# COMP6248-Reproducability-Challenge/selfsupervised-denoising

Measured on AMD Instinct MI355X. Metric: training patches/sec (64x64 gauss25 SSDN), higher is better.
Workload: dtype f16

## Files before the change

### selfsupervised-denoising_amd/csrc/common.h

```cpp
#pragma once
#include <hip/hip_runtime.h>
#include <hip/hip_ext.h>
#include <stdint.h>
#include "../../include/ssdn_hip.h"
#include <cstdlib>

#if defined(SSDN_TUNING)
static inline const char* ssdn_tuning_env(const char* name) { return std::getenv(name); }
#else
static inline const char* ssdn_tuning_env(const char*) { return nullptr; }
#endif

typedef _Float16 h16;
typedef _Float16 half8 __attribute__((ext_vector_type(8)));
typedef _Float16 half4 __attribute__((ext_vector_type(4)));
typedef _Float16 half2v __attribute__((ext_vector_type(2)));
typedef __bf16 bf16x8 __attribute__((ext_vector_type(8)));
typedef unsigned short u16x8 __attribute__((ext_vector_type(8)));
typedef unsigned short u16x4 __attribute__((ext_vector_type(4)));
typedef float f32x16 __attribute__((ext_vector_type(16)));
typedef float f32x4 __attribute__((ext_vector_type(4)));

#define LRELU_SLOPE 0.1f

// ... 111 lines not shown
int launch_adam(const ssdn_adam_args* a, hipStream_t s);
#define ADAM_PACK_MAX 24
int adam_pack_fusable(const ssdn_adam_args* a, const ssdn_wpack_args* const* items, int n);
int launch_adam_pack(const ssdn_adam_args* a, const ssdn_wpack_args* const* items, int n, hipStream_t s);
int launch_metrics(const ssdn_metrics_args* a, hipStream_t s);
int launch_accum(const ssdn_accum_args* a, hipStream_t s);
int launch_noise(const ssdn_noise_args* a, hipStream_t s);
int launch_input_grad(const ssdn_input_grad_args* a, hipStream_t s);
int conv_lds_bytes(const ssdn_conv_args* a);
int conv_validate(const ssdn_conv_args* a);
int chain_len(const ssdn_op* ops, int n, bool any_lane);
int launch_chain(const ssdn_op* ops, int n, bool any_lane, hipStream_t s);
bool chain_merging_on();
bool conv_dma_eligible(const ssdn_conv_args* a, bool any_size);
int conv_dma_lds_bytes(int mt);
bool conv_signs(const ssdn_conv_args* a);
bool gemm_dma_signs(const ssdn_conv_args* a);
bool conv_dma_signs(const ssdn_conv_args* a);
bool conv_fuses_urot(const ssdn_conv_args* a);
bool conv_fuses_unrot(const ssdn_conv_args* a);
bool conv_fuses_upsum(const ssdn_conv_args* a);
bool conv_fuses_pool(const ssdn_conv_args* a);
int launch_conv_dma(const ssdn_conv_args* a, hipStream_t s);
bool conv_thin_eligible(const ssdn_conv_args* a);
bool conv_thin_fuses_pack(const ssdn_pack_input_args* pk, const ssdn_conv_args* a);
int launch_conv_thin(const ssdn_conv_args* a, const ssdn_pack_input_args* pk, hipStream_t s);
bool conv_pack_fusable(const ssdn_pack_input_args* pk, const ssdn_conv_args* a);
bool gradpack_dgrad_fusable(const ssdn_grad_pack_args* gp, const ssdn_conv_args* a);
int launch_gradpack_dgrad(const ssdn_grad_pack_args* gp, const ssdn_conv_args* a, hipStream_t s);
bool conv_gradpack_fusable(const ssdn_grad_pack_args* gp, const ssdn_conv_args* a);
bool gemm_dma_eligible(const ssdn_conv_args* a);
int gemm_dma_lds_bytes(const ssdn_conv_args* a);
int launch_gemm_dma(const ssdn_conv_args* a, hipStream_t s);
bool gemm_dma_fuses_next(const ssdn_conv_args* a, const ssdn_conv_args* b);
int launch_gemm_dma_with_next(const ssdn_conv_args* a, const ssdn_conv_args* b, hipStream_t s);
bool conv_pair_fusable(const ssdn_conv_args* a, const ssdn_conv_args* b);
extern "C" int ssdn_device_cus(void);
int wgrad_lds_bytes(const ssdn_wgrad_args* a);
```

### selfsupervised-denoising_amd/csrc/conv_dma.hip

```cpp
#include "common.h"
#include <cstdlib>
#include <type_traits>
#include <utility>

#if defined(SSDN_CDMA_TUNING) || defined(SSDN_TUNING)
#define CD_ABL(xx, bit) (((xx).ablate & (bit)) != 0)
#define CD_TUNING 1
#else
#define CD_ABL(xx, bit) false
#define CD_TUNING 0
#endif

#ifndef CD_DEPHASE
#define CD_DEPHASE 0
#endif
#ifndef CD_MOVE_BARRIER
#define CD_MOVE_BARRIER 1
#endif
#ifndef CD_WARMUP
#define CD_WARMUP 1
#endif

namespace {

constexpr int CD_TBYTES = 31744;

struct CdAux {
    int m_base, m_cnt;
    int padT, padL, rev;
    int tiles_x, tiles_y;
    int segs, tps;
    int segs_sh;
    unsigned tx_magic;
    int nitems, xcd_map;
    int nfull, tail16;
    int ablate;
    int wrep;
    int dephase;
    unsigned long long* trace;
};

typedef __attribute__((address_space(3))) void* cd_lds_ptr;
__device__ __forceinline__ void dma16(unsigned lds_addr, int voff, __amdgpu_buffer_rsrc_t rs, int soff) {
    __builtin_amdgcn_raw_ptr_buffer_load_lds(rs, (cd_lds_ptr)(size_t)__builtin_amdgcn_readfirstlane(lds_addr), 16, voff, __builtin_amdgcn_readfirstlane(soff), 0, 0);
}

template <bool BF>
__device__ __forceinline__ void cd_mma(f32x16& c, half8 av, half8 bv) {
    if constexpr (BF) c = __builtin_amdgcn_mfma_f32_32x32x16_bf16(__builtin_bit_cast(bf16x8, av), __builtin_bit_cast(bf16x8, bv), c, 0, 0, 0);
    else c = __builtin_amdgcn_mfma_f32_32x32x16_f16(av, bv, c, 0, 0, 0);
}
// ... 46 lines not shown
template <int IMM, int AUX = 0>
__device__ __forceinline__ void dma16i(unsigned lds_addr, int voff, __amdgpu_buffer_rsrc_t rs, int soff) {
    __builtin_amdgcn_raw_ptr_buffer_load_lds(rs, (cd_lds_ptr)(size_t)lds_addr, 16, voff, soff, IMM, AUX);
}

}

template <int MT, bool BF, int EPI, int KIND>
__global__ __launch_bounds__(256, 2) void k_cdma(ssdn_conv_args a, CdAux x) {
    constexpr bool AF = KIND == 1;
    extern __shared__ __attribute__((aligned(16))) char smem[];
    constexpr int WROWS = MT * 32;
    constexpr int WBYTES = WROWS * 96;
    constexpr int OSTR = MT * 64 + 16;
    constexpr int NEK = MT * 2;
    constexpr bool HAS_MASK = (EPI & 1) != 0, HAS_ADD = (EPI & 2) != 0, HAS_UPS = (EPI & 4) != 0, UROT = (EPI & 8) != 0;
    constexpr bool SOUT = (EPI & 16) != 0, SMASK = (EPI & 32) != 0;
    constexpr int NUK = (8 * MT * 4 + 63) / 64;
    constexpr int G = 2 * MT;
    constexpr bool MOVE = CD_MOVE_BARRIER != 0;
    const int tid = threadIdx.x, lane = tid & 63, l31 = lane & 31, kh = lane >> 5;
    const int w = __builtin_amdgcn_readfirstlane(tid >> 6);
    const bool wload = w < 2;
    const int lw = w & 1;
    const unsigned lds0 = (unsigned)(size_t)smem;
    char* const tbuf0 = smem;
    const unsigned tlds0 = lds0, wlds0 = lds0 + 2 * CD_TBYTES;

    const int G_ = gridDim.x;
    int it_first, it_stride, it_end;
    if (x.xcd_map) {
        const int i8 = x.nitems >> 3, xcd = blockIdx.x & 7;
        it_first = xcd * i8 + (blockIdx.x >> 3); it_stride = G_ >> 3; it_end = (xcd + 1) * i8;
    } else {
        it_first = blockIdx.x; it_stride = G_; it_end = x.nitems;
    }
    if (it_first >= it_end) return;
#if CD_WARMUP
    const int pf_line = (blockIdx.x >> 3) * 256 + tid;
    const unsigned pf = __builtin_amdgcn_raw_buffer_load_b32(
        __builtin_amdgcn_make_buffer_rsrc(const_cast<void*>(a.wc), 0, 9 * a.Mpad * a.Ktot * 2, SSDN_BUFFER_RSRC_FLAGS), pf_line << 7, 0, 0);
#endif

    const int bE48 = (4 * w + (l31 >> 4)) * 1728 + (l31 & 15) * 96 + ((kh ^ ((l31 >> 4) & 1)) << 4);
    const int aB48 = l31 * 96 + ((kh ^ ((l31 >> 3) & 1)) << 4);
    const int cpp = x.m_cnt >> 3;

    const __amdgpu_buffer_rsrc_t rs_wc = __builtin_amdgcn_make_buffer_rsrc(const_cast<void*>(a.wc), 0, (int)0x80000000, SSDN_BUFFER_RSRC_FLAGS);
    const int H0 = a.up0 ? (a.H >> 1) : a.H, W0 = a.up0 ? (a.W >> 1) : a.W;
    const int nch = x.nfull + x.tail16;

    int tr_i = 0;
    auto stamp = [&]() __attribute__((always_inline)) {
        if (CD_TUNING && x.trace && tid == 0 && tr_i < 32) x.trace[(size_t)blockIdx.x * 32 + tr_i++] = __builtin_amdgcn_s_memtime();
    };

    const int wtap = a.Mpad * a.Ktot * 2;
    const int wt0 = x.rev ? 8 * wtap : 0, wts = x.rev ? -wtap : wtap;
    const int wvoff = lane * 16;
    const bool lw0 = __builtin_amdgcn_readfirstlane(tid >> 6) == 0;
    auto wchunk = [&](int c) __attribute__((always_inline)) {
        return __builtin_amdgcn_readfirstlane((c * 48 * a.Mpad + x.m_base * ((AF || c < x.nfull) ? 48 : 16)) * 2 + wt0);
    };
    auto wpiece = [&](auto FULLc, auto Jc, unsigned d, int so) __attribute__((always_inline)) {
        using S = CdWSplit<MT, decltype(FULLc)::value != 0>;
        constexpr int j = decltype(Jc)::value;
        if (CD_ABL(x, 2)) return;
        if constexpr (j < S::NB) dma16i<j * 1024>(d, wvoff, rs_wc, so);
        else if constexpr (S::extra) { if (lw0) dma16i<0>(d + 2 * S::NB * 1024, wvoff, rs_wc, so + 2 * S::NB * 1024); }
    };
    auto wbase = [&](bool full) __attribute__((always_inline)) {
        return lw ? (full ? CdWSplit<MT, true>::b1 : CdWSplit<MT, false>::b1) * 1024 : 0;
    };
    auto wslice = [&](bool full, unsigned dbuf, int sl) __attribute__((always_inline)) {
        const int wb = wbase(full);
        if (AF || full) cd_static_for<CdWSplit<MT, true>::NB + 1>([&](auto jc) { wpiece(cd_ic<1>{}, jc, dbuf + wb, sl + wb); });
        else cd_static_for<CdWSplit<MT, false>::NB + 1>([&](auto jc) { wpiece(cd_ic<0>{}, jc, dbuf + wb, sl + wb); });
    };

    __amdgpu_buffer_rsrc_t rs_t = rs_wc;
    int t_so = 0, t_incA = 0, t_incB = 0, t_ybs = 0, rlE = 0, rlO = 0;
    unsigned t_tb = 0;
    auto tile_setup = [&](int tn, int ty0, int tx0, int c, int tbi, bool live) __attribute__((always_inline)) {
        const int k0 = c * 48;
        const bool from0 = k0 < a.c0;
// ... 32 lines not shown
            int voff = (hy & 1) ? rlO : rlE;
            if constexpr (hy < 2 || hy >= 16) voff = (unsigned)(t_ybs + hy) < (unsigned)a.H ? voff : (int)0x80000000;
            if (CD_ABL(x, 512)) dma16i<0, 2>(t_tb + hy * 1728, voff, rs_t, so);
            else dma16i<0>(t_tb + hy * 1728, voff, rs_t, so);
        } else {
            int voff = lw ? rlO : rlE;
            voff = (unsigned)(t_ybs + lw + 2 * hy) < (unsigned)a.H ? voff : (int)0x80000000;
            if (lane < 36) dma16i<0>(t_tb + hy * 1152, voff, rs_t, so);
        }
    };

    auto tile_of = [&](int item, int k) {
        const int strip = item >> x.segs_sh, seg = item & (x.segs - 1);
        CdTile t;
        t.n = x.tiles_x == 1 ? strip : (int)__umulhi((unsigned)strip, x.tx_magic);
        t.x0 = (strip - t.n * x.tiles_x) * 16;
        t.y0 = (seg * x.tps + k) * 16;
        return t;
    };
    int item = it_first, kt = 0;
    CdTile cur = tile_of(item, 0);
    int tpar = 0, wpar = 0;
    float* const bl = reinterpret_cast<float*>(smem + 18 * 18 * 96);
    if (tid < WROWS) bl[tid] = (a.bias && tid < x.m_cnt) ? a.bias[x.m_base + tid] : 0.f;
    constexpr int CD_LUT = 18 * 18 * 96 + 384;
    static_assert(CD_LUT + 256 <= CD_TBYTES && WROWS * 4 <= 384, "pad behind tile buffer 0");
    if constexpr (SMASK && HAS_MASK) {
        if (tid < 64) reinterpret_cast<float*>(smem + CD_LUT)[tid] = ((tid >> 2) >> (tid & 3)) & 1 ? 1.f : LRELU_SLOPE;
    }

    const __amdgpu_buffer_rsrc_t rs_dst = __builtin_amdgcn_make_buffer_rsrc(UROT ? a.urot.p : a.dst.p, 0, CD_ABL(x, 64) ? 0 : (int)0x80000000, SSDN_BUFFER_RSRC_FLAGS);
    const __amdgpu_buffer_rsrc_t rs_sgn = __builtin_amdgcn_make_buffer_rsrc(SOUT ? a.sign_out : a.urot_smask, 0, (!CD_ABL(x, 64) && (SOUT || (UROT && a.urot_smask))) ? (int)0x80000000 : 0, SSDN_BUFFER_RSRC_FLAGS);
    const __amdgpu_buffer_rsrc_t rs_ms = __builtin_amdgcn_make_buffer_rsrc(const_cast<void*>(HAS_UPS ? a.upsum_mask_sign : a.mask_sign), 0, SMASK ? (int)0x80000000 : 0, SSDN_BUFFER_RSRC_FLAGS);
    const float slope = a.act ? LRELU_SLOPE : 1.f;
    const __amdgpu_buffer_rsrc_t rs_mask = __builtin_amdgcn_make_buffer_rsrc(a.mask.p, 0, HAS_MASK ? (int)0x80000000 : 0, SSDN_BUFFER_RSRC_FLAGS);
    const __amdgpu_buffer_rsrc_t rs_add = __builtin_amdgcn_make_buffer_rsrc(a.add.p, 0, HAS_ADD ? (int)0x80000000 : 0, SSDN_BUFFER_RSRC_FLAGS);
    const __amdgpu_buffer_rsrc_t rs_up = __builtin_amdgcn_make_buffer_rsrc(a.upsum.p, 0, HAS_UPS ? (int)0x80000000 : 0, SSDN_BUFFER_RSRC_FLAGS);
    const __amdgpu_buffer_rsrc_t rs_um = __builtin_amdgcn_make_buffer_rsrc(a.upsum_mask.p, 0, HAS_UPS ? (int)0x80000000 : 0, SSDN_BUFFER_RSRC_FLAGS);
    int u_pc[NUK];
#pragma unroll
    for (int k = 0; k < NUK; ++k) {
        const int p = k * 64 + lane;
        const int j = p / cpp, c = p - j * cpp;
        u_pc[k] = p < 8 * cpp ? (j | (c << 8)) : -1;
    }

    auto run = [&](auto WLc) __attribute__((always_inline)) {
// ... 164 lines not shown
        if (!CD_ABL(x, 8) && !HAS_UPS && (cpp & 1) == 0 && !CD_ABL(x, 1024)) {
            const int pix_t = (cur.n * a.H + cur.y0 + 4 * w) * a.W + cur.x0;
            const int npair = __builtin_amdgcn_readfirstlane(cpp >> 1);
            int lane_o = lane;
            asm volatile("" : "+v"(lane_o));
            const int l31 = lane_o & 31, kh = lane_o >> 5;
            const int lrow = l31 >> 4, lcol = l31 & 15;
            const int lpix = lrow * a.W + lcol;
            int ur_base = 0, ur_iu = 0, ur_iv = 0, ur_ju = 0, ur_jv = 0;
            if constexpr (UROT) {
                const int Bq = a.N >> 2, P1 = a.H - 1;
                const int r = (cur.n >= Bq ? 1 : 0) + (cur.n >= 2 * Bq ? 1 : 0) + (cur.n >= 3 * Bq ? 1 : 0);
                ur_iu = r == 0 ? 1 : (r == 2 ? -1 : 0); ur_iv = r == 1 ? 1 : (r == 3 ? -1 : 0);
                ur_ju = r == 3 ? 1 : (r == 1 ? -1 : 0); ur_jv = r == 0 ? 1 : (r == 2 ? -1 : 0);
                const int i0 = r >= 2 ? P1 : 0, j0 = (r == 1 || r == 2) ? P1 : 0;
                ur_base = (((cur.n - r * Bq) * a.H + i0) * a.W + j0) * a.urot.cs + a.urot.co + r * a.M;
            }
            constexpr bool HOIST = HAS_MASK && SMASK && !HAS_ADD && !UROT;
            unsigned mbh[2][MT * 2];
            if constexpr (HOIST) {
#pragma unroll
                for (int nt = 0; nt < 2; ++nt) {
                    const int pix_p = pix_t + 2 * nt * a.W;
                    const int s_so = __builtin_amdgcn_readfirstlane(pix_p * (a.M >> 3) + (x.m_base >> 3));
#pragma unroll
                    for (int i = 0; i < MT * 2; ++i) {
                        if (i >= npair) break;
                        mbh[nt][i] = __builtin_amdgcn_raw_buffer_load_b8(rs_ms, lpix * (a.M >> 3) + kh + i * 2, s_so, 0);
                    }
                }
            }
            auto pass = [&](auto NtC, auto ActC) __attribute__((always_inline)) {
                constexpr int nt = decltype(NtC)::value;
                constexpr bool ACTC = decltype(ActC)::value != 0;
                const int pix_p = pix_t + 2 * nt * a.W;
                int d_lane, d_so = 0;
                bool live = true;
                if constexpr (UROT) {
                    const int u = cur.y0 + 4 * w + 2 * nt + lrow + 1, v = cur.x0 + lcol;
                    live = u < a.H;
                    const int dpx = (ur_iu * u + ur_iv * v) * a.W + ur_ju * u + ur_jv * v;
                    d_lane = live ? (ur_base + dpx * a.urot.cs + x.m_base) * 2 + kh * 16 : (int)0x80000000;
                } else {
                    d_lane = lpix * a.dst.cs * 2 + kh * 16;
                    d_so = __builtin_amdgcn_readfirstlane((pix_p * a.dst.cs + a.dst.co + x.m_base) * 2);
                }
                const int s_lane = live ? lpix * (a.M >> 3) + kh : (int)0x80000000;
                const int s_so = __builtin_amdgcn_readfirstlane(pix_p * (a.M >> 3) + (x.m_base >> 3));
                u32x4_t ab[MT * 2], mb[MT * 2];
#pragma unroll
                for (int i = 0; i < MT * 2; ++i) {
                    if (i >= npair) break;
                    if constexpr (HAS_ADD)
                        ab[i] = __builtin_amdgcn_raw_buffer_load_b128(rs_add, lpix * a.add.cs * 2 + kh * 16 + i * 32,
                                                                      __builtin_amdgcn_readfirstlane((pix_p * a.add.cs + a.add.co + x.m_base) * 2), 0);
                    if constexpr (HOIST)
                        mb[i][0] = mbh[nt][i];
                    else if constexpr (HAS_MASK && SMASK)
                        mb[i][0] = __builtin_amdgcn_raw_buffer_load_b8(rs_ms, s_lane + i * 2, s_so, 0);
                    else if constexpr (HAS_MASK)
                        mb[i] = __builtin_amdgcn_raw_buffer_load_b128(rs_mask, lpix * a.mask.cs * 2 + kh * 16 + i * 32,
                                                                      __builtin_amdgcn_readfirstlane((pix_p * a.mask.cs + a.mask.co + x.m_base) * 2), 0);
                }
#pragma unroll
                for (int mt = 0; mt < MT; ++mt)
#pragma unroll
                    for (int gp = 0; gp < 2; ++gp) {
                        constexpr int DUMMY = 0; (void)DUMMY;
                        const int i = mt * 2 + gp;
                        if (i >= npair) break;
                        unsigned pk[2][2];
#pragma unroll
                        for (int h = 0; h < 2; ++h) {
                            float v[4];
#pragma unroll
                            for (int j = 0; j < 4; ++j) v[j] = acc[mt][nt][(2 * gp + h) * 4 + j];
                            if constexpr (ACTC) {
#pragma unroll
                                for (int j = 0; j < 4; j += 2) {
                                    const f32x2_t t = f32x2_t{v[j], v[j + 1]} * LRELU_SLOPE;
                                    asm("v_max_f32 %0, %1, %2" : "=v"(v[j]) : "v"(v[j]), "v"(t[0]));
                                    asm("v_max_f32 %0, %1, %2" : "=v"(v[j + 1]) : "v"(v[j + 1]), "v"(t[1]));
                                }
                            }
                            pk[h][0] = BF ? pack_bf16x2(v[0], v[1]) : pack_f16x2(v[0], v[1]);
// ... 83 lines not shown
                const int Bq = a.N >> 2, P1 = a.H - 1;
                const int r = (cur.n >= Bq ? 1 : 0) + (cur.n >= 2 * Bq ? 1 : 0) + (cur.n >= 3 * Bq ? 1 : 0);
                ur_iu = r == 0 ? 1 : (r == 2 ? -1 : 0); ur_iv = r == 1 ? 1 : (r == 3 ? -1 : 0);
                ur_ju = r == 3 ? 1 : (r == 1 ? -1 : 0); ur_jv = r == 0 ? 1 : (r == 2 ? -1 : 0);
                const int i0 = r >= 2 ? P1 : 0, j0 = (r == 1 || r == 2) ? P1 : 0;
                ur_base = (((cur.n - r * Bq) * a.H + i0) * a.W + j0) * a.urot.cs + a.urot.co + r * a.M;
            }
#pragma unroll
            for (int nt = 0; nt < 2; ++nt) {
                const int pix_p = pix_t + 2 * nt * a.W;
                u32x4_t ab[NEK], mb[NEK];
                int goff[NEK], soff[NEK];
#pragma unroll
                for (int k = 0; k < NEK; ++k) {
                    int epc = e_pc[k];
                    asm volatile("" : "+v"(epc));
                    const bool on = epc >= 0;
                    const int px = epc & 255, c16 = (epc >> 8) << 4;
                    const int pix = pix_p + (px >> 4) * a.W + (px & 15);
                    if constexpr (UROT) {
                        const int u = cur.y0 + 4 * w + 2 * nt + (px >> 4) + 1, v = cur.x0 + (px & 15);
                        const bool live = on && u < a.H;
                        const int dpx = (ur_iu * u + ur_iv * v) * a.W + ur_ju * u + ur_jv * v;
                        goff[k] = live ? (ur_base + dpx * a.urot.cs + x.m_base) * 2 + c16 : (int)0x80000000;
                        soff[k] = live ? pix * (a.M >> 3) + (x.m_base >> 3) + (c16 >> 4) : (int)0x80000000;
                    } else
                    goff[k] = on ? (pix * a.dst.cs + a.dst.co + x.m_base) * 2 + c16 : (int)0x80000000;
                    if constexpr (HAS_ADD)
                        ab[k] = __builtin_amdgcn_raw_buffer_load_b128(rs_add, on ? (pix * a.add.cs + a.add.co + x.m_base) * 2 + c16 : (int)0x80000000, 0, 0);
                    if constexpr (HAS_MASK && SMASK)
                        mb[k][0] = __builtin_amdgcn_raw_buffer_load_b8(rs_ms, on ? pix * (a.M >> 3) + (x.m_base >> 3) + (c16 >> 4) : (int)0x80000000, 0, 0);
                    else if constexpr (HAS_MASK)
                        mb[k] = __builtin_amdgcn_raw_buffer_load_b128(rs_mask, on ? (pix * a.mask.cs + a.mask.co + x.m_base) * 2 + c16 : (int)0x80000000, 0, 0);
                    if constexpr (SOUT) soff[k] = on ? pix * (a.M >> 3) + (x.m_base >> 3) + (c16 >> 4) : (int)0x80000000;
                }
#pragma unroll
                for (int mt = 0; mt < MT; ++mt)
#pragma unroll
                    for (int gp = 0; gp < 2; ++gp) {
                        unsigned pk[2][2];
#pragma unroll
                        for (int h = 0; h < 2; ++h) {
                            float v[4];
#pragma unroll
                            for (int j = 0; j < 4; ++j) v[j] = acc[mt][nt][(2 * gp + h) * 4 + j];
                            if constexpr (!BF) {
#pragma unroll
                                for (int j = 0; j < 4; j += 2) {
                                    const f32x2_t t = f32x2_t{v[j], v[j + 1]} * slope;
                                    asm("v_max_f32 %0, %1, %2" : "=v"(v[j]) : "v"(v[j]), "v"(t[0]));
                                    asm("v_max_f32 %0, %1, %2" : "=v"(v[j + 1]) : "v"(v[j + 1]), "v"(t[1]));
                                }
                            }
                            pk[h][0] = BF ? pack_bf16x2(v[0], v[1]) : pack_f16x2(v[0], v[1]);
                            pk[h][1] = BF ? pack_bf16x2(v[2], v[3]) : pack_f16x2(v[2], v[3]);
                        }
                        u32x4_t o;
#pragma unroll
                        for (int d = 0; d < 2; ++d) {
                            auto r = __builtin_amdgcn_permlane32_swap(pk[0][d], pk[1][d], false, false);
                            o[d] = r[0]; o[2 + d] = r[1];
                        }
                        const int piece = mt * 4 + 2 * gp + kh;
                        *reinterpret_cast<u32x4_t*>(reg + l31 * OSTR + piece * 16) = o;
                    }
                if constexpr (HAS_UPS) {
                    const int pixl = (cur.n * (a.H >> 1) + ((cur.y0 + 4 * w + 2 * nt) >> 1)) * (a.W >> 1) + (cur.x0 >> 1);
                    u32x4_t um[NUK];
#pragma unroll
                    for (int k = 0; k < NUK; ++k) {
                        int upc = u_pc[k];
                        asm volatile("" : "+v"(upc));
                        const bool on = upc >= 0;
                        const int j = upc & 255, c16 = (upc >> 8) << 4;
                        if constexpr (SMASK)
                            um[k][0] = __builtin_amdgcn_raw_buffer_load_b8(rs_ms, on ? (pixl + j) * (a.upsum_c >> 3) + (x.m_base >> 3) + (c16 >> 4) : (int)0x80000000, 0, 0);
                        else
                        um[k] = __builtin_amdgcn_raw_buffer_load_b128(rs_um, on ? ((pixl + j) * a.upsum_mask.cs + a.upsum_mask.co + x.m_base) * 2 + c16 : (int)0x80000000, 0, 0);
                    }
#pragma unroll
                    for (int k = 0; k < NUK; ++k) {
                        int upc = u_pc[k];
                        asm volatile("" : "+v"(upc));
                        const bool on = upc >= 0;
                        const int j = upc & 255, c16 = (upc >> 8) << 4;
                        float sum[8] = {0.f, 0.f, 0.f, 0.f, 0.f, 0.f, 0.f, 0.f};
#pragma unroll
                        for (int q4 = 0; q4 < 4; ++q4) {
                            const u32x4_t o = *reinterpret_cast<const u32x4_t*>(reg + (on ? ((q4 >> 1) * 16 + 2 * j + (q4 & 1)) * OSTR + c16 : 0));
#pragma unroll
                            for (int q = 0; q < 4; ++q) { sum[2 * q] += bf_lo(o[q]); sum[2 * q + 1] += bf_hi(o[q]); }
                        }
                        u32x4_t r;
#pragma unroll
                        for (int q = 0; q < 4; ++q) {
                            int mlo, mhi;
                            if constexpr (SMASK) { mlo = (um[k][0] >> (2 * q)) & 1u; mhi = (um[k][0] >> (2 * q + 1)) & 1u; }
                            else { mlo = (int)(short)(um[k][q] & 0xffffu); mhi = (int)um[k][q] >> 16; }
                            r[q] = pack_bf16x2(sum[2 * q] * (mlo > 0 ? 1.f : LRELU_SLOPE), sum[2 * q + 1] * (mhi > 0 ? 1.f : LRELU_SLOPE));
                        }
                        __builtin_amdgcn_raw_buffer_store_b128(r, rs_up, on ? ((pixl + j) * a.upsum.cs + a.upsum.co + x.m_base) * 2 + c16 : (int)0x80000000, 0, 0);
                    }
                } else {
#pragma unroll
                for (int k = 0; k < NEK; ++k) {
                    int epc = e_pc[k];
                    asm volatile("" : "+v"(epc));
                    const bool on = epc >= 0;
                    const int px = epc & 255, c16 = (epc >> 8) << 4;
                    u32x4_t o = *reinterpret_cast<const u32x4_t*>(reg + (on ? px * OSTR + c16 : 0));
                    if constexpr (HAS_MASK || HAS_ADD) {
#pragma unroll
                        for (int q = 0; q < 4; ++q) {
                            float v0, v1;
                            if constexpr (BF) {
                                v0 = bf_lo(o[q]); v1 = bf_hi(o[q]);
                                if constexpr (HAS_ADD) { v0 += bf_lo(ab[k][q]); v1 += bf_hi(ab[k][q]); }
                            } else {
                                v0 = f16_lo(o[q]); v1 = f16_hi(o[q]);
                                if constexpr (HAS_ADD) { v0 += f16_lo(ab[k][q]); v1 += f16_hi(ab[k][q]); }
                            }
                            if constexpr (HAS_MASK) {
                                int mlo, mhi;
                                if constexpr (SMASK) { mlo = (mb[k][0] >> (2 * q)) & 1u; mhi = (mb[k][0] >> (2 * q + 1)) & 1u; }
// ... 42 lines not shown
        if (i != 2 - t / 3 || j != 2 - t % 3) mir = false;
    }
    if (!fwd && !mir) return false;
    *padT = -mny; *padL = -mnx; *rev = fwd ? 0 : 1;
    return true;
}

bool conv_dma_eligible(const ssdn_conv_args* a, bool any_size) {
    int pt, pl, rv;
    if (!cd_window(a, &pt, &pl, &rv)) return false;
    if (a->dst32 || (a->H & 15) || (a->W & 15) || !a->wc) return false;
    const int tail = a->Ktot % 48;
    if (tail != 0 && tail != 16) return false;
    if (a->c0 % 48 && a->c0 != a->Ktot) return false;
    if ((a->M & 7) || (a->Mpad & 31)) return false;
    if (!a->bf16 && (a->mask.p || a->add.p)) return false;
    if (a->bf16 && a->act) return false;
    if (a->urot.p && (a->bf16 || a->M != 96 || a->Mpad != 96 || a->H != a->W || (a->N & 3) || a->mask.p || a->add.p || a->upsum.p || a->pool.p ||
                      (a->urot.co & 7) || (a->urot.cs & 7) || (long long)(a->N / 4) * a->H * a->W * a->urot.cs * 2 >= (1ll << 31))) return false;
    if (a->upsum.p && (!a->bf16 || a->mask.p || a->add.p || a->upsum_c % 96 || a->upsum_c > a->M)) return false;
    int cus = ssdn_device_cus();
    if (cus <= 0) cus = 256;
    const long long tiles = (long long)a->N * (a->H >> 4) * (a->W >> 4);
    if (!(tiles >= cus || (2 * tiles >= cus && a->H * a->W > 256)) && !any_size) return false;
    if ((long long)a->N * (a->W >> 4) >= 65536) return false;
    int csmax = a->dst.cs > a->src1.cs ? a->dst.cs : a->src1.cs;
    csmax = csmax > a->src0.cs ? csmax : a->src0.cs;
    csmax = csmax > a->mask.cs ? csmax : a->mask.cs;
    csmax = csmax > a->add.cs ? csmax : a->add.cs;
    if ((long long)a->N * a->H * a->W * csmax * 2 >= (1ll << 31)) return false;
    if (9ll * a->Mpad * a->Ktot * 2 >= (1ll << 31)) return false;
    return true;
}

bool conv_dma_signs(const ssdn_conv_args* a) {
    if (!conv_dma_eligible(a, false)) return false;
    if (a->sign_out && (a->bf16 || !a->dst.p || a->urot.p || a->M != 96 || a->Mpad != 96)) return false;
    if (a->mask_sign && (!a->bf16 || !a->mask.p || a->add.p || a->upsum.p || a->mask.cs != a->M || a->mask.co != 0 || (a->Mpad != 96 && a->Mpad != 64))) return false;
    if (a->upsum_mask_sign && (!a->bf16 || !a->upsum.p || a->upsum_mask.cs != a->upsum_c || a->upsum_mask.co != 0)) return false;
    return true;
}

int conv_dma_lds_bytes(int mt) { return 2 * CD_TBYTES + 2 * mt * 32 * 96; }

template <int MT, bool BF, int EPI, int KIND>
static int cd_launch_kind(const ssdn_conv_args* a, CdAux x, hipStream_t s) {
    static bool attr_set_dev[SSDN_MAX_DEVICES_ATTR] = {};
    bool& attr_set = attr_set_dev[ssdn_current_device_slot()];
    if (!attr_set) {
        SSDN_CHECK_HIP(hipFuncSetAttribute((const void*)k_cdma<MT, BF, EPI, KIND>, hipFuncAttributeMaxDynamicSharedMemorySize, 160 * 1024));
        attr_set = true;
    }
    int cus = ssdn_device_cus();
    if (cus <= 0) return -1;
    const int nstrips = a->N * x.tiles_x;
    x.segs = 1;
    while (nstrips * x.segs < 2 * cus && x.segs < x.tiles_y && x.tiles_y % (x.segs * 2) == 0) x.segs *= 2;
    x.tps = x.tiles_y / x.segs;
    x.segs_sh = 0;
    while ((1 << x.segs_sh) < x.segs) ++x.segs_sh;
    x.tx_magic = x.tiles_x > 1 ? (unsigned)((0x100000000ull + x.tiles_x - 1) / x.tiles_x) : 0u;
    x.nitems = nstrips * x.segs;
    const int grid = x.nitems < 2 * cus ? x.nitems : 2 * cus;
    x.xcd_map = (x.nitems % 8 == 0 && grid % 8 == 0) ? 1 : 0;
    const double px = (double)a->N * a->H * a->W;
    const int kreal = a->kreal > 0 ? a->kreal : a->Ktot;
    const double flops = 2.0 * px * x.m_cnt * kreal * 9;
    const double bytes = px * (a->c0 * 2.0 / (a->up0 ? 4.0 : 1.0) + a->c1 * 2.0) + px * x.m_cnt * 2.0;
    prof_begin(MT == 3 ? SSDN_PROF_CDMA_MT3 : SSDN_PROF_CDMA_MT21, s);
    SSDN_LAUNCH((k_cdma<MT, BF, EPI, KIND>), dim3(grid), dim3(256), conv_dma_lds_bytes(MT), s, *a, x);
    prof_end(MT == 3 ? SSDN_PROF_CDMA_MT3 : SSDN_PROF_CDMA_MT21, s, flops, bytes);
    return 0;
}
template <int MT, bool BF, int EPI>
static int cd_launch(const ssdn_conv_args* a, const CdAux& x, hipStream_t s) {
    if (x.tail16 == 0 && x.nfull > 0) return cd_launch_kind<MT, BF, EPI, 1>(a, x, s);
    if constexpr (!BF) {
        if (x.tail16 == 1 && x.nfull > 0) return cd_launch_kind<MT, BF, EPI, 2>(a, x, s);
    }
    return cd_launch_kind<MT, BF, EPI, 0>(a, x, s);
}

template <int MT>
static int cd_launch_role(const ssdn_conv_args* a, const CdAux& x, hipStream_t s) {
    if (a->urot.p) {
        if constexpr (MT == 3) return cd_launch<3, false, 8>(a, x, s);
        return ssdn_set_error("conv_dma: fused UNROT_FWD needs M = 96");
    }
    if (!a->bf16) {
        if (a->sign_out) {
            if constexpr (MT == 3) return cd_launch<3, false, 16>(a, x, s);
            return ssdn_set_error("conv_dma: sign_out needs M = 96");
        }
// ... 3 lines not shown
        if constexpr (MT == 3) {
            if (x.m_base + 96 <= a->upsum_c && x.m_cnt == 96 && !a->mask.p && !a->add.p)
                return a->upsum_mask_sign ? cd_launch<3, true, 4 | 32>(a, x, s) : cd_launch<3, true, 4>(a, x, s);
        }
        return ssdn_set_error("conv_dma: fused upsum needs whole 96-channel blocks without mask / add");
    }
    const int epi = (a->mask.p ? 1 : 0) | (a->add.p ? 2 : 0);
    if (a->mask_sign) {
        if constexpr (MT >= 2) { if (epi == 1) return cd_launch<MT, true, 1 | 32>(a, x, s); }
        return ssdn_set_error("conv_dma: mask_sign needs a mask, no skip gradient, Mpad = 96 or 64");
    }
    switch (epi) {
        case 0: return cd_launch<MT, true, 0>(a, x, s);
        case 1: return cd_launch<MT, true, 1>(a, x, s);
        case 2: return cd_launch<MT, true, 2>(a, x, s);
        default: return cd_launch<MT, true, 3>(a, x, s);
    }
}

int launch_conv_dma(const ssdn_conv_args* a, hipStream_t s) {
    CdAux x;
    if (!cd_window(a, &x.padT, &x.padL, &x.rev)) return ssdn_set_error("conv_dma: not a 3x3 window");
    x.tiles_x = a->W >> 4; x.tiles_y = a->H >> 4;
    x.segs = 1; x.tps = x.tiles_y; x.nitems = 0; x.xcd_map = 0; x.segs_sh = 0; x.tx_magic = 0;
    x.nfull = a->Ktot / 48; x.tail16 = (a->Ktot % 48) ? 1 : 0;
    static const int env_ablate = [] { const char* e = ssdn_tuning_env("SSDN_CDMA_ABLATE"); return e ? atoi(e) : 0; }();
    x.ablate = env_ablate;
    static const int env_wrep = [] { const char* e = ssdn_tuning_env("SSDN_CDMA_WREP"); return e ? atoi(e) : 0; }();
    x.wrep = env_wrep;
    static const int env_dephase = [] { const char* e = ssdn_tuning_env("SSDN_CDMA_DEPHASE"); return e ? atoi(e) : CD_DEPHASE; }();
    x.dephase = env_dephase;
    x.trace = (unsigned long long*)ssdn_debug_get_trace();
    int rc = 0;
    for (int mb = 0; mb < a->Mpad && !rc; mb += 96) {
        int rows = a->Mpad - mb;
        rows = rows > 96 ? 96 : rows;
        const int mt = rows / 32;
        x.m_base = mb;
        x.m_cnt = a->M - mb < rows ? a->M - mb : rows;
        if (x.m_cnt <= 0) break;
        if (mt == 3) rc = cd_launch_role<3>(a, x, s);
        else if (mt == 2) rc = cd_launch_role<2>(a, x, s);
        else rc = cd_launch_role<1>(a, x, s);
    }
    if (rc) return rc;
    SSDN_CHECK_HIP(hipGetLastError());
    return 0;
}

#endif
```

### selfsupervised-denoising_amd/csrc/conv_mfma.hip

```cpp
#include "common.h"
#ifdef SSDN_TUNING
#define CV_ABL(xx, bit) (((xx).ablate & (bit)) != 0)
#define CV_TUNING 1
#else
#define CV_ABL(xx, bit) false
#define CV_TUNING 0
#endif
#include <cstdlib>


struct ConvGeom {
    int TW, TH, TN, HH, HW, padT, padB, padL, padR;
    int PSTR, WSTR, NP;
    int tiles_x, tiles_y, groups_n;
};

static __host__ __device__ inline ConvGeom conv_geom(int ltw, int lth, int ltn, int ntaps, const int* dy, const int* dx,
                                                     int N, int H, int W, int kc) {
    ConvGeom g;
    g.TW = 1 << ltw; g.TH = 1 << lth; g.TN = 1 << ltn;
    int mny = 0, mxy = 0, mnx = 0, mxx = 0;
    for (int t = 0; t < ntaps; ++t) {
        mny = dy[t] < mny ? dy[t] : mny; mxy = dy[t] > mxy ? dy[t] : mxy;
        mnx = dx[t] < mnx ? dx[t] : mnx; mxx = dx[t] > mxx ? dx[t] : mxx;
// ... 634 lines not shown
                        v1 *= lrelu_grad(f16_hi(mb[w]));
                    }
                    o[w] = BF ? pack_bf16x2(v0, v1) : pack_f16x2(v0, v1);
                }
            }
            __builtin_amdgcn_raw_buffer_store_b128(o, rd[u], go[u], 0, 0);
        }
    }
    stamp();
}

static bool conv_uses_mt1(const ssdn_conv_args* a, const ConvGeom& g) {
    static int mt1_tiles = -1;
    if (mt1_tiles < 0) {
        const char* e = ssdn_tuning_env("SSDN_CONV_MT1_TILES");
        mt1_tiles = e ? atoi(e) : ssdn_device_cus();
        if (mt1_tiles <= 0) mt1_tiles = 256;
    }
    return !a->dst32 && g.tiles_x * g.tiles_y * g.groups_n <= mt1_tiles && a->Mpad >= 64;
}

static int g_conv_mode = [] { const char* e = ssdn_tuning_env("SSDN_CONV_DMA"); return e ? atoi(e) : 1; }();
extern "C" int ssdn_conv_set_mode(int mode) {
    if (mode < 0 || mode > 2) return ssdn_set_error("conv mode must be 0, 1 or 2");
    g_conv_mode = mode;
    return 0;
}
static bool conv_use_dma(const ssdn_conv_args* a) { return g_conv_mode > 0 && !a->pool.p && conv_dma_eligible(a, g_conv_mode == 2); }
static bool conv_use_gemm(const ssdn_conv_args* a) { return g_conv_mode > 0 && gemm_dma_eligible(a); }
static bool conv_use_thin(const ssdn_conv_args* a) { return g_conv_mode > 0 && conv_thin_eligible(a); }
bool conv_gradpack_fusable(const ssdn_grad_pack_args* gp, const ssdn_conv_args* a) {
    return !conv_validate(a) && !conv_use_gemm(a) && !conv_use_thin(a) && !conv_use_dma(a) && gradpack_dgrad_fusable(gp, a);
}
bool conv_pair_fusable(const ssdn_conv_args* a, const ssdn_conv_args* b) {
    return !conv_validate(a) && !conv_validate(b) && conv_use_gemm(a) && gemm_dma_fuses_next(a, b);
}
bool conv_pack_fusable(const ssdn_pack_input_args* pk, const ssdn_conv_args* a) {
    return !conv_validate(a) && !conv_use_gemm(a) && conv_use_thin(a) && conv_thin_fuses_pack(pk, a);
}

int conv_validate(const ssdn_conv_args* a) {
    if (a->ntaps < 1 || a->ntaps > SSDN_MAX_TAPS) return ssdn_set_error("conv: ntaps out of range");
    if (a->ltw + a->lth + a->ltn > 9 || a->ltw < 0 || a->lth < 0 || a->ltn < 0) return ssdn_set_error("conv: tile must have <= 512 pixels");
    if (a->Ktot != a->c0 + a->c1 || (a->Ktot & 15)) return ssdn_set_error("conv: Ktot must equal c0+c1 and be a multiple of 16");
    if ((a->c0 & 7) || (a->c1 & 7)) return ssdn_set_error("conv: source channel counts must be multiples of 8");
    if (a->kc < 16 || (a->kc & 15) || a->Ktot % a->kc || (a->kc > 64 && a->kc != 96)) return ssdn_set_error("conv: kc must be 16, 32, 48, 64 or 96 and divide Ktot");
    if ((a->Mpad & 31) || a->M > a->Mpad) return ssdn_set_error("conv: Mpad must be a multiple of 32 and >= M");
    if (!a->dst32 && ((a->M & 7) || (a->dst.co & 7) || (a->dst.cs & 7))) return ssdn_set_error("conv: 16-bit output needs M, dst.co, dst.cs %% 8 == 0");
    if (a->add.p && ((a->add.co & 7) || (a->add.cs & 7))) return ssdn_set_error("conv: add view must be 16-byte aligned");
    if (a->mask.p && ((a->mask.co & 7) || (a->mask.cs & 7))) return ssdn_set_error("conv: mask view must be 16-byte aligned");
// ... 164 lines not shown
```

### selfsupervised-denoising_amd/ssdn/hip/graph.py

```python
from __future__ import annotations

import os
from dataclasses import dataclass, field
from typing import Dict, List, Optional, Set, Tuple

LDS_LIMIT = 160 * 1024
CONV_LDS_PREFERRED = 80 * 1024
WGRAD_SMALL_PX = 32768
SMALL_WGRAD_G, SMALL_WGRAD_CUS = 2, 64
MID_WGRAD_PX, MID_WGRAD_G = 131072, 2
WGRAD_CU_FRAC = (3, 4)
WGRAD_MEGA = "split"
FUSE_UNROT_FWD = True
SIGN_BYTES_HEAD = True
X16_SLOTS = 16
POOL_ROUTE = True
SIGN_BYTES_CONV = True
SIGN_BYTES = True
MEGA_MIN_PX = 32768
SPLIT_HEAD_CUS = (1, 2)
SPLIT_AFTER = "decode_block_2.2"
SPLIT_GROUP0 = ("output_block", "decode_block_2.2")
MEGA_LANE = 0
WGRAD_LANE = 1
# ... 146 lines not shown


def _behind_runs(at: Dict[int, int], runs, only=None) -> None:
    for first, end in runs:
        for k in at:
            if first <= at[k] < end and (only is None or k in only):
                at[k] = end



def _pads(taps):
    dys = [t[0] for t in taps]
    dxs = [t[1] for t in taps]
    return max(0, -min(dys)), max(0, max(dys)), max(0, -min(dxs)), max(0, max(dxs))


def _pow2ceil_log(v: int) -> int:
    l = 0
    while (1 << l) < v:
        l += 1
    return l


def cdma_fills(tiles: int, cus: int, H: int = 0, W: int = 0) -> bool:
    return tiles >= cus or (2 * tiles >= cus and H * W > 256)


def choose_conv_tile(N, H, W, taps, Ktot, Mpad, budget=LDS_LIMIT, out16=True, cus=256):
    padT, padB, padL, padR = _pads(taps)
    best = None
    for ltw in range(0, min(5, _pow2ceil_log(W)) + 1):
        for lth in range(0, min(8 - ltw, _pow2ceil_log(H)) + 1):
            for ltn in range(0, min(8 - ltw - lth, _pow2ceil_log(N)) + 1):
                TW, TH, TN = 1 << ltw, 1 << lth, 1 << ltn
                tiles = -(-W // TW) * -(-H // TH) * -(-N // TN)
                util = (N * H * W) / (tiles * 256.0)
                NP = TN * (TH + padT + padB) * (TW + padL + padR)
                mt1 = out16 and tiles <= cus and Mpad >= 64
                mt = 1 if mt1 else min(3, Mpad // 32)
                kcs = [kc for kc in ((16, 32, 48, 64, 96) if mt1 else (16, 32, 48, 64)) if Ktot % kc == 0]
                for kc in kcs:
                    lds = NP * (kc * 2 + 16) + 2 * mt * 32 * (kc * 2 + 16)
                    if len(taps) == 1 and Ktot // kc >= 2:
                        lds = max(lds, 2 * NP * kc * 2 + 2 * mt * 32 * (kc * 2 + 16))
                    if out16:
                        lds = max(lds, TN * TH * TW * (mt * 64 + 16) + mt * 128)
                    if lds > budget:
                        continue
# ... 594 lines not shown
```

Measured before the change: 20570.

## Split M=96 forward DMA conv across grid.y to fill CUs on small grids

Adds an output-channel split for plain M=96 forward convs in the DMA conv kernel: when too few spatial strips exist to fill twice the CU count, it launches an MT=1 kernel with three blocks in grid.y, each handling 32 output rows. It also relaxes DMA-conv eligibility for f16 (non-bf16) convs to require only 2*tiles >= CUs, so more small layers take this path. The aim is better CU occupancy on low-resolution layers, at the cost of rereading input tiles three times and using a narrower MMA tile per block. A Python helper mirrors the relaxed eligibility, and a new conv mode 3 disables the split.

```diff
diff --git a/selfsupervised-denoising_amd/csrc/common.h b/selfsupervised-denoising_amd/csrc/common.h
--- a/selfsupervised-denoising_amd/csrc/common.h
+++ b/selfsupervised-denoising_amd/csrc/common.h
@@ -157,6 +157,7 @@
 bool conv_fuses_upsum(const ssdn_conv_args* a);
 bool conv_fuses_pool(const ssdn_conv_args* a);
 int launch_conv_dma(const ssdn_conv_args* a, hipStream_t s);
+int conv_mode_now();
 bool conv_thin_eligible(const ssdn_conv_args* a);
 bool conv_thin_fuses_pack(const ssdn_pack_input_args* pk, const ssdn_conv_args* a);
 int launch_conv_thin(const ssdn_conv_args* a, const ssdn_pack_input_args* pk, hipStream_t s);
diff --git a/selfsupervised-denoising_amd/csrc/conv_dma.hip b/selfsupervised-denoising_amd/csrc/conv_dma.hip
--- a/selfsupervised-denoising_amd/csrc/conv_dma.hip
+++ b/selfsupervised-denoising_amd/csrc/conv_dma.hip
@@ -27,6 +27,7 @@
 
 struct CdAux {
     int m_base, m_cnt;
+    int msplit;
     int padT, padL, rev;
     int tiles_x, tiles_y;
     int segs, tps;
@@ -119,6 +120,7 @@
     const int tid = threadIdx.x, lane = tid & 63, l31 = lane & 31, kh = lane >> 5;
     const int w = __builtin_amdgcn_readfirstlane(tid >> 6);
     const bool wload = w < 2;
+    const int m_base = MT == 1 ? x.m_base + (int)blockIdx.y * 32 : x.m_base;
     const int lw = w & 1;
     const unsigned lds0 = (unsigned)(size_t)smem;
     char* const tbuf0 = smem;
@@ -157,7 +159,7 @@
     const int wvoff = lane * 16;
     const bool lw0 = __builtin_amdgcn_readfirstlane(tid >> 6) == 0;
     auto wchunk = [&](int c) __attribute__((always_inline)) {
-        return __builtin_amdgcn_readfirstlane((c * 48 * a.Mpad + x.m_base * ((AF || c < x.nfull) ? 48 : 16)) * 2 + wt0);
+        return __builtin_amdgcn_readfirstlane((c * 48 * a.Mpad + m_base * ((AF || c < x.nfull) ? 48 : 16)) * 2 + wt0);
     };
     auto wpiece = [&](auto FULLc, auto Jc, unsigned d, int so) __attribute__((always_inline)) {
         using S = CdWSplit<MT, decltype(FULLc)::value != 0>;
@@ -236,7 +238,7 @@
     CdTile cur = tile_of(item, 0);
     int tpar = 0, wpar = 0;
     float* const bl = reinterpret_cast<float*>(smem + 18 * 18 * 96);
-    if (tid < WROWS) bl[tid] = (a.bias && tid < x.m_cnt) ? a.bias[x.m_base + tid] : 0.f;
+    if (tid < WROWS) bl[tid] = (a.bias && tid < x.m_cnt) ? a.bias[m_base + tid] : 0.f;
     constexpr int CD_LUT = 18 * 18 * 96 + 384;
     static_assert(CD_LUT + 256 <= CD_TBYTES && WROWS * 4 <= 384, "pad behind tile buffer 0");
     if constexpr (SMASK && HAS_MASK) {
@@ -447,7 +449,7 @@
 #pragma unroll
                 for (int nt = 0; nt < 2; ++nt) {
                     const int pix_p = pix_t + 2 * nt * a.W;
-                    const int s_so = __builtin_amdgcn_readfirstlane(pix_p * (a.M >> 3) + (x.m_base >> 3));
+                    const int s_so = __builtin_amdgcn_readfirstlane(pix_p * (a.M >> 3) + (m_base >> 3));
 #pragma unroll
                     for (int i = 0; i < MT * 2; ++i) {
                         if (i >= npair) break;
@@ -465,27 +467,27 @@
                     const int u = cur.y0 + 4 * w + 2 * nt + lrow + 1, v = cur.x0 + lcol;
                     live = u < a.H;
                     const int dpx = (ur_iu * u + ur_iv * v) * a.W + ur_ju * u + ur_jv * v;
-                    d_lane = live ? (ur_base + dpx * a.urot.cs + x.m_base) * 2 + kh * 16 : (int)0x80000000;
+                    d_lane = live ? (ur_base + dpx * a.urot.cs + m_base) * 2 + kh * 16 : (int)0x80000000;
                 } else {
                     d_lane = lpix * a.dst.cs * 2 + kh * 16;
-                    d_so = __builtin_amdgcn_readfirstlane((pix_p * a.dst.cs + a.dst.co + x.m_base) * 2);
+                    d_so = __builtin_amdgcn_readfirstlane((pix_p * a.dst.cs + a.dst.co + m_base) * 2);
                 }
                 const int s_lane = live ? lpix * (a.M >> 3) + kh : (int)0x80000000;
-                const int s_so = __builtin_amdgcn_readfirstlane(pix_p * (a.M >> 3) + (x.m_base >> 3));
+                const int s_so = __builtin_amdgcn_readfirstlane(pix_p * (a.M >> 3) + (m_base >> 3));
                 u32x4_t ab[MT * 2], mb[MT * 2];
 #pragma unroll
                 for (int i = 0; i < MT * 2; ++i) {
                     if (i >= npair) break;
                     if constexpr (HAS_ADD)
                         ab[i] = __builtin_amdgcn_raw_buffer_load_b128(rs_add, lpix * a.add.cs * 2 + kh * 16 + i * 32,
-                                                                      __builtin_amdgcn_readfirstlane((pix_p * a.add.cs + a.add.co + x.m_base) * 2), 0);
+                                                                      __builtin_amdgcn_readfirstlane((pix_p * a.add.cs + a.add.co + m_base) * 2), 0);
                     if constexpr (HOIST)
                         mb[i][0] = mbh[nt][i];
                     else if constexpr (HAS_MASK && SMASK)
                         mb[i][0] = __builtin_amdgcn_raw_buffer_load_b8(rs_ms, s_lane + i * 2, s_so, 0);
                     else if constexpr (HAS_MASK)
                         mb[i] = __builtin_amdgcn_raw_buffer_load_b128(rs_mask, lpix * a.mask.cs * 2 + kh * 16 + i * 32,
-                                                                      __builtin_amdgcn_readfirstlane((pix_p * a.mask.cs + a.mask.co + x.m_base) * 2), 0);
+                                                                      __builtin_amdgcn_readfirstlane((pix_p * a.mask.cs + a.mask.co + m_base) * 2), 0);
                 }
 #pragma unroll
                 for (int mt = 0; mt < MT; ++mt)
@@ -615,17 +617,17 @@
                         const int u = cur.y0 + 4 * w + 2 * nt + (px >> 4) + 1, v = cur.x0 + (px & 15);
                         const bool live = on && u < a.H;
                         const int dpx = (ur_iu * u + ur_iv * v) * a.W + ur_ju * u + ur_jv * v;
-                        goff[k] = live ? (ur_base + dpx * a.urot.cs + x.m_base) * 2 + c16 : (int)0x80000000;
-                        soff[k] = live ? pix * (a.M >> 3) + (x.m_base >> 3) + (c16 >> 4) : (int)0x80000000;
+                        goff[k] = live ? (ur_base + dpx * a.urot.cs + m_base) * 2 + c16 : (int)0x80000000;
+                        soff[k] = live ? pix * (a.M >> 3) + (m_base >> 3) + (c16 >> 4) : (int)0x80000000;
                     } else
-                    goff[k] = on ? (pix * a.dst.cs + a.dst.co + x.m_base) * 2 + c16 : (int)0x80000000;
+                    goff[k] = on ? (pix * a.dst.cs + a.dst.co + m_base) * 2 + c16 : (int)0x80000000;
                     if constexpr (HAS_ADD)
-                        ab[k] = __builtin_amdgcn_raw_buffer_load_b128(rs_add, on ? (pix * a.add.cs + a.add.co + x.m_base) * 2 + c16 : (int)0x80000000, 0, 0);
+                        ab[k] = __builtin_amdgcn_raw_buffer_load_b128(rs_add, on ? (pix * a.add.cs + a.add.co + m_base) * 2 + c16 : (int)0x80000000, 0, 0);
                     if constexpr (HAS_MASK && SMASK)
-                        mb[k][0] = __builtin_amdgcn_raw_buffer_load_b8(rs_ms, on ? pix * (a.M >> 3) + (x.m_base >> 3) + (c16 >> 4) : (int)0x80000000, 0, 0);
+                        mb[k][0] = __builtin_amdgcn_raw_buffer_load_b8(rs_ms, on ? pix * (a.M >> 3) + (m_base >> 3) + (c16 >> 4) : (int)0x80000000, 0, 0);
                     else if constexpr (HAS_MASK)
-                        mb[k] = __builtin_amdgcn_raw_buffer_load_b128(rs_mask, on ? (pix * a.mask.cs + a.mask.co + x.m_base) * 2 + c16 : (int)0x80000000, 0, 0);
-                    if constexpr (SOUT) soff[k] = on ? pix * (a.M >> 3) + (x.m_base >> 3) + (c16 >> 4) : (int)0x80000000;
+                        mb[k] = __builtin_amdgcn_raw_buffer_load_b128(rs_mask, on ? (pix * a.mask.cs + a.mask.co + m_base) * 2 + c16 : (int)0x80000000, 0, 0);
+                    if constexpr (SOUT) soff[k] = on ? pix * (a.M >> 3) + (m_base >> 3) + (c16 >> 4) : (int)0x80000000;
                 }
 #pragma unroll
                 for (int mt = 0; mt < MT; ++mt)
@@ -667,9 +669,9 @@
                         const bool on = upc >= 0;
                         const int j = upc & 255, c16 = (upc >> 8) << 4;
                         if constexpr (SMASK)
-                            um[k][0] = __builtin_amdgcn_raw_buffer_load_b8(rs_ms, on ? (pixl + j) * (a.upsum_c >> 3) + (x.m_base >> 3) + (c16 >> 4) : (int)0x80000000, 0, 0);
+                            um[k][0] = __builtin_amdgcn_raw_buffer_load_b8(rs_ms, on ? (pixl + j) * (a.upsum_c >> 3) + (m_base >> 3) + (c16 >> 4) : (int)0x80000000, 0, 0);
                         else
-                        um[k] = __builtin_amdgcn_raw_buffer_load_b128(rs_um, on ? ((pixl + j) * a.upsum_mask.cs + a.upsum_mask.co + x.m_base) * 2 + c16 : (int)0x80000000, 0, 0);
+                        um[k] = __builtin_amdgcn_raw_buffer_load_b128(rs_um, on ? ((pixl + j) * a.upsum_mask.cs + a.upsum_mask.co + m_base) * 2 + c16 : (int)0x80000000, 0, 0);
                     }
 #pragma unroll
                     for (int k = 0; k < NUK; ++k) {
@@ -692,7 +694,7 @@
                             else { mlo = (int)(short)(um[k][q] & 0xffffu); mhi = (int)um[k][q] >> 16; }
                             r[q] = pack_bf16x2(sum[2 * q] * (mlo > 0 ? 1.f : LRELU_SLOPE), sum[2 * q + 1] * (mhi > 0 ? 1.f : LRELU_SLOPE));
                         }
-                        __builtin_amdgcn_raw_buffer_store_b128(r, rs_up, on ? ((pixl + j) * a.upsum.cs + a.upsum.co + x.m_base) * 2 + c16 : (int)0x80000000, 0, 0);
+                        __builtin_amdgcn_raw_buffer_store_b128(r, rs_up, on ? ((pixl + j) * a.upsum.cs + a.upsum.co + m_base) * 2 + c16 : (int)0x80000000, 0, 0);
                     }
                 } else {
 #pragma unroll
@@ -781,7 +783,8 @@
     int cus = ssdn_device_cus();
     if (cus <= 0) cus = 256;
     const long long tiles = (long long)a->N * (a->H >> 4) * (a->W >> 4);
-    if (!(tiles >= cus || (2 * tiles >= cus && a->H * a->W > 256)) && !any_size) return false;
+    const bool fills = a->bf16 ? (tiles >= cus || (2 * tiles >= cus && a->H * a->W > 256)) : 2 * tiles >= cus;
+    if (!fills && !any_size) return false;
     if ((long long)a->N * (a->W >> 4) >= 65536) return false;
     int csmax = a->dst.cs > a->src1.cs ? a->dst.cs : a->src1.cs;
     csmax = csmax > a->src0.cs ? csmax : a->src0.cs;
@@ -802,6 +805,13 @@
 
 int conv_dma_lds_bytes(int mt) { return 2 * CD_TBYTES + 2 * mt * 32 * 96; }
 
+static int cd_segments(const ssdn_conv_args* a, const CdAux& x, int cus) {
+    const int nstrips = a->N * x.tiles_x;
+    int segs = 1;
+    while (nstrips * segs < 2 * cus && segs < x.tiles_y && x.tiles_y % (segs * 2) == 0) segs *= 2;
+    return segs;
+}
+
 template <int MT, bool BF, int EPI, int KIND>
 static int cd_launch_kind(const ssdn_conv_args* a, CdAux x, hipStream_t s) {
     static bool attr_set_dev[SSDN_MAX_DEVICES_ATTR] = {};
@@ -812,9 +822,8 @@
     }
     int cus = ssdn_device_cus();
     if (cus <= 0) return -1;
+    x.segs = cd_segments(a, x, cus);
     const int nstrips = a->N * x.tiles_x;
-    x.segs = 1;
-    while (nstrips * x.segs < 2 * cus && x.segs < x.tiles_y && x.tiles_y % (x.segs * 2) == 0) x.segs *= 2;
     x.tps = x.tiles_y / x.segs;
     x.segs_sh = 0;
     while ((1 << x.segs_sh) < x.segs) ++x.segs_sh;
@@ -824,10 +833,11 @@
     x.xcd_map = (x.nitems % 8 == 0 && grid % 8 == 0) ? 1 : 0;
     const double px = (double)a->N * a->H * a->W;
     const int kreal = a->kreal > 0 ? a->kreal : a->Ktot;
-    const double flops = 2.0 * px * x.m_cnt * kreal * 9;
-    const double bytes = px * (a->c0 * 2.0 / (a->up0 ? 4.0 : 1.0) + a->c1 * 2.0) + px * x.m_cnt * 2.0;
+    const int m_all = x.m_cnt * (MT == 1 ? x.msplit : 1);
+    const double flops = 2.0 * px * m_all * kreal * 9;
+    const double bytes = px * (a->c0 * 2.0 / (a->up0 ? 4.0 : 1.0) + a->c1 * 2.0) + px * m_all * 2.0;
     prof_begin(MT == 3 ? SSDN_PROF_CDMA_MT3 : SSDN_PROF_CDMA_MT21, s);
-    SSDN_LAUNCH((k_cdma<MT, BF, EPI, KIND>), dim3(grid), dim3(256), conv_dma_lds_bytes(MT), s, *a, x);
+    SSDN_LAUNCH((k_cdma<MT, BF, EPI, KIND>), dim3(grid, MT == 1 ? x.msplit : 1), dim3(256), conv_dma_lds_bytes(MT), s, *a, x);
     prof_end(MT == 3 ? SSDN_PROF_CDMA_MT3 : SSDN_PROF_CDMA_MT21, s, flops, bytes);
     return 0;
 }
@@ -877,7 +887,7 @@
     CdAux x;
     if (!cd_window(a, &x.padT, &x.padL, &x.rev)) return ssdn_set_error("conv_dma: not a 3x3 window");
     x.tiles_x = a->W >> 4; x.tiles_y = a->H >> 4;
-    x.segs = 1; x.tps = x.tiles_y; x.nitems = 0; x.xcd_map = 0; x.segs_sh = 0; x.tx_magic = 0;
+    x.segs = 1; x.tps = x.tiles_y; x.nitems = 0; x.xcd_map = 0; x.segs_sh = 0; x.tx_magic = 0; x.msplit = 1;
     x.nfull = a->Ktot / 48; x.tail16 = (a->Ktot % 48) ? 1 : 0;
     static const int env_ablate = [] { const char* e = ssdn_tuning_env("SSDN_CDMA_ABLATE"); return e ? atoi(e) : 0; }();
     x.ablate = env_ablate;
@@ -887,6 +897,17 @@
     x.dephase = env_dephase;
     x.trace = (unsigned long long*)ssdn_debug_get_trace();
     int rc = 0;
+    const bool plain = !a->urot.p && !a->sign_out && !a->mask_sign && !a->upsum_mask_sign && !a->upsum.p && !a->mask.p && !a->add.p && !a->pool.p;
+    if (plain && a->M == 96 && a->Mpad == 96 && conv_mode_now() != 3) {
+        int cus = ssdn_device_cus();
+        if (cus > 0 && (long long)a->N * x.tiles_x * cd_segments(a, x, cus) < 2ll * cus) {
+            x.m_base = 0; x.m_cnt = 32; x.msplit = 3;
+            rc = cd_launch_role<1>(a, x, s);
+            if (rc) return rc;
+            SSDN_CHECK_HIP(hipGetLastError());
+            return 0;
+        }
+    }
     for (int mb = 0; mb < a->Mpad && !rc; mb += 96) {
         int rows = a->Mpad - mb;
         rows = rows > 96 ? 96 : rows;
diff --git a/selfsupervised-denoising_amd/csrc/conv_mfma.hip b/selfsupervised-denoising_amd/csrc/conv_mfma.hip
--- a/selfsupervised-denoising_amd/csrc/conv_mfma.hip
+++ b/selfsupervised-denoising_amd/csrc/conv_mfma.hip
@@ -680,10 +680,11 @@
 
 static int g_conv_mode = [] { const char* e = ssdn_tuning_env("SSDN_CONV_DMA"); return e ? atoi(e) : 1; }();
 extern "C" int ssdn_conv_set_mode(int mode) {
-    if (mode < 0 || mode > 2) return ssdn_set_error("conv mode must be 0, 1 or 2");
+    if (mode < 0 || mode > 3) return ssdn_set_error("conv mode must be 0, 1, 2 or 3");
     g_conv_mode = mode;
     return 0;
 }
+int conv_mode_now() { return g_conv_mode; }
 static bool conv_use_dma(const ssdn_conv_args* a) { return g_conv_mode > 0 && !a->pool.p && conv_dma_eligible(a, g_conv_mode == 2); }
 static bool conv_use_gemm(const ssdn_conv_args* a) { return g_conv_mode > 0 && gemm_dma_eligible(a); }
 static bool conv_use_thin(const ssdn_conv_args* a) { return g_conv_mode > 0 && conv_thin_eligible(a); }
diff --git a/selfsupervised-denoising_amd/ssdn/hip/graph.py b/selfsupervised-denoising_amd/ssdn/hip/graph.py
--- a/selfsupervised-denoising_amd/ssdn/hip/graph.py
+++ b/selfsupervised-denoising_amd/ssdn/hip/graph.py
@@ -192,8 +192,19 @@
     return l
 
 
-def cdma_fills(tiles: int, cus: int, H: int = 0, W: int = 0) -> bool:
+def cdma_fills(tiles: int, cus: int, H: int = 0, W: int = 0, fwd: bool = False) -> bool:
+    if fwd:
+        return 2 * tiles >= cus
     return tiles >= cus or (2 * tiles >= cus and H * W > 256)
+
+
+def cdma_serves_op(a: dict, cus: int) -> bool:
+    H, W = a["H"], a["W"]
+    if len(a["taps"]) != 9 or H % 16 or W % 16 or a.get("dst32") is not None or a.get("pool") is not None:
+        return False
+    if a["Ktot"] % 48 not in (0, 16) or (a["c0"] % 48 and a["c0"] != a["Ktot"]) or a["M"] % 8:
+        return False
+    return cdma_fills(a["N"] * (H // 16) * (W // 16), cus, H, W, fwd=a["role"] == "fwd")
 
 
 def choose_conv_tile(N, H, W, taps, Ktot, Mpad, budget=LDS_LIMIT, out16=True, cus=256):
```

New measurement: 20760 (median of 6 runs). No clear change (+0.9%).
